# liyangSKD/slam-eslam

Measured on AMD Instinct MI355X. Metric: M particle-updates/s (predict+weight+resample) @ 1/2/4/8 MI355X, higher is better.
Workload: dtype f64; 1 GPU; configs[2]: 4194304 particles/GPU, 1 MI355X per rank, MLS 1000x1000 @0.1 m, 4 contacts, resample forced every step; particles_per_gpu=4194304, global_particles=4194304, parallelism=dp1 (particle shards)

## Files before the change

### include/eslam_detmath.h

```cpp
#ifndef ESLAM_DETMATH_H
#define ESLAM_DETMATH_H

#include <stdint.h>

#if defined(__HIPCC__)
#define DM_FN __host__ __device__ static inline __attribute__((always_inline))
#define DM_CONST static constexpr
#define DM_UNROLL _Pragma("unroll")
#else
#define DM_FN static inline
#define DM_CONST static const
#define DM_UNROLL
#endif

DM_FN uint64_t dm_bits(double x) { uint64_t u; __builtin_memcpy(&u, &x, 8); return u; }
DM_FN double dm_from_bits(uint64_t u) { double x; __builtin_memcpy(&x, &u, 8); return x; }
DM_FN uint32_t dm_fbits(float x) { uint32_t u; __builtin_memcpy(&u, &x, 4); return u; }
DM_FN int dm_isnan(double x) { return x != x; }
DM_FN int dm_isfinite(double x) { return (dm_bits(x) & 0x7ff0000000000000ull) != 0x7ff0000000000000ull; }
DM_FN double dm_fabs(double x) { return dm_from_bits(dm_bits(x) & 0x7fffffffffffffffull); }
DM_FN double dm_fma(double a, double b, double c) { return __builtin_fma(a, b, c); }
#if defined(__HIP_DEVICE_COMPILE__)
DM_FN double dm_fmak(double a, double b, double k)
{
// ... 1380 lines not shown
    uint64_t b = dm_bits(v);
    int e = (int)(b >> 52);
    if (e == 0x7ff) return 0x3fffffffffffffffull;
    if (e == 0) return 0;
    uint64_t m = (b & 0x000fffffffffffffull) | 0x0010000000000000ull;
    int sh = e - 1075 + shift;
    if (sh >= 10) return 0x3fffffffffffffffull;
    if (sh >= 0) return m << sh;
    if (sh <= -64) return 0;
    return m >> (-sh);
}

DM_FN uint64_t dm_fx61(double v) { return dm_fx_shift(v, 61); }

DM_FN uint64_t dm_count_draws_le(uint64_t c, uint64_t N, uint32_t xs, int shift)
{
    const unsigned __int128 prod = (unsigned __int128)c * N;
    const uint64_t kstar = (uint64_t)(prod >> shift);
    const uint64_t k0 = kstar >= 1 ? kstar - 1 : 0;
    if (k0 >= N) return N;
    uint64_t cnt = k0;
    uint32_t x = dm_mulmod31(dm_minstd_pow(k0 + 1), xs);
    const double dN = (double)N;
    for (uint64_t k = k0; k <= kstar + 1 && k < N; ++k) {
        const double u = dm_minstd_uniform(x);
        const uint64_t T = dm_fx_shift(((double)k + u) / dN, shift);
        if (T <= c) cnt = k + 1;
        else break;
        x = dm_minstd_next(x);
    }
    return cnt;
}


DM_FN int dm_fx128_limbs(double v, int scale, uint32_t limb[4])
{
    limb[0] = limb[1] = limb[2] = limb[3] = 0;
    if (!(v > 0.0)) return 0;
    uint64_t b = dm_bits(v);
    int e = (int)(b >> 52);
    uint64_t m;
    int ex;
    if (e == 0) { m = b & 0x000fffffffffffffull; ex = -1074; }
    else { m = (b & 0x000fffffffffffffull) | 0x0010000000000000ull; ex = e - 1075; }
    int sh = ex + scale;
    unsigned __int128 x;
    if (sh >= 0) {
        if (sh > 74) { limb[0] = limb[1] = limb[2] = 0xffffffffu; limb[3] = 0x7fffffffu; return 1; }
        x = (unsigned __int128)m << sh;
    } else {
        if (sh <= -64) return 0;
        x = (unsigned __int128)(m >> (-sh));
    }
    limb[0] = (uint32_t)x;
    limb[1] = (uint32_t)(x >> 32);
    limb[2] = (uint32_t)(x >> 64);
    limb[3] = (uint32_t)(x >> 96);
    return 0;
}

DM_FN double dm_limbs_to_double(const uint64_t L[4], int scale)
{
    uint32_t d[6];
    uint64_t carry = 0;
    for (int j = 0; j < 4; ++j) {
        uint64_t lo = (L[j] & 0xffffffffull) + carry;
// ... 307 lines not shown
```

### include/eslam_gpu.h

```cpp
#ifndef ESLAM_GPU_H
#define ESLAM_GPU_H

#include <stddef.h>
#include <stdint.h>

#ifdef __cplusplus
extern "C" {
#endif

#define ESLAM_ABI_VERSION 8

#define ESLAM_MAX_CONTACTS 32

#define ESLAM_OK 0
#define ESLAM_ERR_INVALID_ARG -1
#define ESLAM_ERR_NO_ENVIRONMENT -2
#define ESLAM_ERR_ZERO_MEAS_VAR -3
#define ESLAM_ERR_HASH_SAMPLE -4
#define ESLAM_ERR_NO_MLS_GRID -5
#define ESLAM_ERR_HIP -6
#define ESLAM_ERR_NOT_INITIALISED -7
#define ESLAM_ERR_UNSUPPORTED -8
#define ESLAM_ERR_OUT_OF_MEMORY -9
#define ESLAM_ERR_COMM -10
// ... 193 lines not shown

int eslam_gpu_scan_from_laser(eslam_ctx* ctx, const eslam_laser_scan* scan, const eslam_scan_params* params,
                              eslam_scan_info* info);
int eslam_gpu_scan_from_depth(eslam_ctx* ctx, const eslam_depth_image* image, const eslam_scan_params* params,
                              eslam_scan_info* info);
int eslam_gpu_scan_patches(eslam_ctx* ctx, eslam_scan_patch* out, uint64_t capacity, uint64_t* count);

typedef struct eslam_cpoint {
    double point[3];
    double zdiff, zvar;
    double prob;
} eslam_cpoint;

typedef struct eslam_particle_record {
    double position[2];
    double orientation, zpos, zsigma, mprob, weight;
    double meas_pos[3];
    double meas_theta;
    uint64_t index;
    uint32_t n_cpoints;
    uint8_t floating;
    uint8_t pad[3];
} eslam_particle_record;

int eslam_gpu_download_records(eslam_ctx* ctx, uint64_t first, uint64_t stride, uint64_t count,
                               eslam_particle_record* out, eslam_cpoint* cpoints, uint32_t max_cpoints);
int eslam_gpu_particle_count(const eslam_ctx* ctx, uint64_t* n);

int eslam_gpu_step(eslam_ctx* ctx, const eslam_step_input* in, int* updated);
int eslam_gpu_project(eslam_ctx* ctx, const eslam_step_input* in);
int eslam_gpu_update(eslam_ctx* ctx, const eslam_step_input* in);
int eslam_gpu_sync(eslam_ctx* ctx, eslam_update_info* info);
int eslam_gpu_debug_set_spin_limit(eslam_ctx* ctx, uint32_t polls);

int eslam_gpu_get_weights_sum(eslam_ctx* ctx, double* sum);
int eslam_gpu_normalize_weights(eslam_ctx* ctx, double* effective);
int eslam_gpu_resample(eslam_ctx* ctx);
typedef struct {
    uint64_t n_before;
    uint64_t n_after;
    uint64_t overruns;
    uint64_t dropped;
} eslam_resample_info;
int eslam_gpu_resample_stratified(eslam_ctx* ctx, uint64_t samples, eslam_resample_info* info);
int eslam_gpu_resample_multinomial(eslam_ctx* ctx, uint64_t samples, eslam_resample_info* info);
int eslam_gpu_get_best_particle_index(eslam_ctx* ctx, uint64_t* index);
int eslam_gpu_get_centroid(eslam_ctx* ctx, double position[3], double orientation[4]);

typedef struct eslam_rng_state {
    uint32_t minstd_x;
    uint32_t pad;
    uint64_t project_count;
    uint64_t init_count;
    uint64_t hash_count;
    double max_weight;
    double ud_pose[12];
    uint32_t libc_rand[34];
    uint32_t libc_rand_pos;
    uint32_t pad2;
} eslam_rng_state;
int eslam_gpu_get_rng_state(eslam_ctx* ctx, eslam_rng_state* st);
int eslam_gpu_set_rng_state(eslam_ctx* ctx, const eslam_rng_state* st);

#define ESLAM_SNAPSHOT_VERSION 1
#define ESLAM_SNAPSHOT_GRID 0x1u
#define ESLAM_SNAPSHOT_HASH 0x2u
// ... 71 lines not shown
```

### slam-eslam_amd/csrc/eslam_ctx.hip

```cpp
#include <hip/hip_runtime.h>
#include <rccl/rccl.h>
#include <dlfcn.h>

#include <math.h>
#include <stdlib.h>
#include <stdio.h>
#include <string.h>

#include <string>
#include <chrono>
#include <algorithm>
#include <atomic>
#include <functional>
#include <vector>

#include "eslam_internal.h"
#include "eslam_launch.h"
#include "eslam_buf.h"

using namespace eslam_dev;
using namespace eslam_buf;

namespace {

// ... 175 lines not shown

struct eslam_ctx {
    eslam_config cfg;
    int device = 0;
    hipStream_t stream = nullptr;
    bool own_stream = false;
    uint64_t n = 0, cap = 0;
    uint64_t gbase = 0, n_global = 0;
    DevState st[2] = {};
    ParticleBufs pt;
    uint64_t* fin_word = nullptr;
    uint32_t pub_stride = 0;
    uint64_t fin_epoch = 0;
    uint32_t scan_tag = 0;
    bool has_anc = false;
    LocalMaps lm = {};
    LocalMapBufs lmb;
    bool lm_ready = false;
    Pinned<ScanPatch> scan_host[2];
    Dev<ScanPatch> scan_dev[2];
    Event scan_ev[2];
    uint32_t scan_slot = 0;
    DebugRec dbg = {};
    DebugBufs dbgb;
    uint64_t dbg_cap = 0;
    bool dbg_valid = false;
    Dev<Shard> shards;
    Dev<Ctl> ctl;
    Pinned<Ctl> ctl_host;
    Pinned<uint32_t> fault_host;
    bool poisoned = false;
    bool poison_pages = false;
    uint32_t spin_limit = kSpinLimit;
    Dev<uint32_t> jump;
    uint32_t jump_n = 1;
    uint64_t jump_n_for = 0;
    Dev<double> scratch;
    Pinned<double> scratch_host;
    bool has_map = false;
    MapView map = {};
    GridBufs grid;
    uint64_t map_np = 0;
    uint64_t map_np_cap = 0;
    Dev<void> sm_mem;
    Dev<void> sm_x;
    Dev<void> pg_mem;
    GridBufs pg_out;
    uint64_t pg_out_cap = 0, pg_out_cells = 0;
    Dev<void> scan_mem;
    Dev<eslam_scan_patch> scan_out;
    uint64_t scan_count = 0;
    Pinned<void> snap_host[2];
    Dev<void> snap_dev[2];
    uint64_t snap_cap = 0;
    Event snap_ev[2];
    uint32_t maxp = 4;
    uint64_t proj_event = 0, init_event = 0, hash_event = 0;
    double ud_pose[12];
    double zcomp[4] = {1, 0, 0, 0};
    bool sharded = false;
    bool statics_sharded = false;
    eslam_comm comm = {};
    std::vector<uint64_t> gall;
    Dev<Shard> recs;
    Dev<uint64_t> mg;
    void* rccl = nullptr;
// ... 2069 lines not shown
    const double motion = sqrt(p.mu[0] * p.mu[0] + p.mu[1] * p.mu[1]) +
                          6.0 * sqrt(in->sample_cov[0] + in->sample_cov[4]);
    p.win_margin = reach + motion + 0.05;
    p.use_window = (c.flags & ESLAM_FLAG_NO_MAP_LDS) ? 0u : 1u;
    p.me2 = c.measurement_error * c.measurement_error;
    p.radius = c.contact_point_radius;
    p.corr = c.contact_likelihood_correction;
    p.min_contacts = c.min_contacts;
    p.use_shape = c.use_shape_update ? 1u : 0u;
    p.use_slip = c.use_slip_update ? 1u : 0u;
    p.n = ctx->n;
    p.gbase = ctx->gbase;
    p.n_global = ctx->n_global;
    p.J = dm_chunk_rows_cfg(ctx->n_global, ctx->cfg.sum_chunk_rows);
}

static uint32_t scan_items(uint64_t n)
{
    if (n <= (1ull << 18)) return 1u;
    return n <= (1ull << 19) ? 2u : (n <= (2ull << 20) ? 4u : (uint32_t)kScanItems);
}

static ScanParams scan_params(eslam_ctx* ctx, uint32_t phase_b, uint32_t normalize, bool multi)
{
    ScanParams sp;
    memset(&sp, 0, sizeof(sp));
    sp.spin_limit = ctx->spin_limit;
    sp.fault = ctx->fault_host;
    sp.n = ctx->n;
    sp.gbase = ctx->gbase;
    sp.n_global = ctx->n_global;
    sp.phase_b = phase_b;
    sp.normalize = normalize;
    sp.items = multi ? (uint32_t)kScanItems : scan_items(ctx->n);
    const uint64_t tile = (uint64_t)kBlock * sp.items;
    sp.ntiles = (uint32_t)((ctx->n + tile - 1) / tile);
    sp.pub_stride = ctx->pub_stride;
    return sp;
}

static FinParams fin_params(eslam_ctx* ctx, uint32_t mode)
{
    FinParams fp;
    memset(&fp, 0, sizeof(fp));
    fp.n_global = ctx->n_global;
    fp.min_effective = ctx->cfg.min_effective;
    fp.discount = ctx->cfg.discount_factor;
    fp.spread_threshold = ctx->cfg.spread_threshold;
    fp.mode = mode;
    if (ctx->jump_n_for != ctx->n_global) {
        ctx->jump_n = dm_minstd_pow(ctx->n_global);
        ctx->jump_n_for = ctx->n_global;
    }
    fp.minstd_jump_n = ctx->jump_n;
    return fp;
}

static int abort_pending_gather(eslam_ctx* ctx, hipError_t e, int rc = ESLAM_ERR_HIP)
{
    if (e != hipSuccess) fail(ctx, ESLAM_ERR_HIP, (std::string("sharded resample: ") + hipGetErrorString(e)).c_str());
    (void)hipMemsetAsync(ctx->pt.marks, 0, ctx->cap * 4, ctx->stream);
    (void)hipMemsetAsync(&ctx->ctl->flip, 0, sizeof(uint32_t), ctx->stream);
    (void)hipMemsetAsync(&ctx->ctl->gather, 0, sizeof(uint32_t), ctx->stream);
    (void)hipStreamSynchronize(ctx->stream);
    return rc;
}

// ... 439 lines not shown
    return launch_step(ctx, in, true, false);
}

extern "C" int eslam_gpu_update(eslam_ctx* ctx, const eslam_step_input* in)
{
    if (!ctx || !in) return ESLAM_ERR_INVALID_ARG;
    return launch_step(ctx, in, false, true);
}

extern "C" int eslam_gpu_step(eslam_ctx* ctx, const eslam_step_input* in, int* updated)
{
    if (!ctx || !in) return ESLAM_ERR_INVALID_ARG;
    const bool gate = update_gate(ctx->cfg.measurement_threshold_distance, ctx->cfg.measurement_threshold_angle, ctx->ud_pose,
                                  in->body2odometry_rot, in->body2odometry_trans) ||
                      in->ltc_count > 0;
    const int rc = launch_step(ctx, in, true, gate);
    if (rc) return rc;
    if (gate) {
        double R[9];
        q_to_mat(in->body2odometry_rot, R);
        for (int r = 0; r < 3; ++r) {
            for (int c = 0; c < 3; ++c) ctx->ud_pose[r * 4 + c] = R[r * 3 + c];
            ctx->ud_pose[r * 4 + 3] = in->body2odometry_trans[r];
        }
    }
    if (updated) *updated = gate ? 1 : 0;
    return ESLAM_OK;
}

extern "C" int eslam_gpu_debug_set_spin_limit(eslam_ctx* ctx, uint32_t polls)
{
    if (!ctx) return ESLAM_ERR_INVALID_ARG;
    ctx->spin_limit = polls;
    return ESLAM_OK;
}

extern "C" int eslam_gpu_sync(eslam_ctx* ctx, eslam_update_info* info)
{
    if (!ctx) return ESLAM_ERR_INVALID_ARG;
    if (const int rc_ = settle(ctx)) return rc_;
    int rc = read_ctl(ctx);
    if (rc) return rc;
    const Ctl& c = *ctx->ctl_host;
    if (info) {
        info->effective = c.eff;
        info->weight_sum = c.S;
        info->floating_weight = c.fw;
        info->max_weight = c.max_weight;
        info->data_particles = c.data_particles;
        info->total_points = c.total_points;
        info->resampled = (int32_t)c.resample;
        info->uniform_reset = (int32_t)c.uniform;
        info->resample_overruns = c.overruns;
        info->update_count = c.update_count;
        info->map_patches_dropped = c.map_dropped;
        info->map_stores_copied = c.map_copied;
        info->map_patches_covered = c.map_covered;
        info->map_stores_changed = c.map_changed;
        info->map_cells_written = c.map_written;
        info->map_pages_taken = c.map_taken;
        info->map_tiles_evicted = c.map_evicted;
        info->map_pages_free = c.pg_nfree > c.pg_cursor ? c.pg_nfree - c.pg_cursor : 0;
    }
    double acc[5];
    eslam_kernel_times& t = ctx->times;
    if (const uint32_t steps = ctx->timing ? ctx->ring.sums(acc) : 0) {
// ... 1426 lines not shown
```

### slam-eslam_amd/csrc/eslam_kernels.hip

```cpp
#include <hip/hip_runtime.h>
#include <type_traits>
#include <string.h>

#include "eslam_internal.h"
#include "eslam_launch.h"

namespace eslam_dev {

template <int O> __device__ __forceinline__ uint32_t xor_lane_u32(uint32_t v)
{
    static_assert(O == 1 || O == 2 || O == 4 || O == 8 || O == 16 || O == 32, "xor distance");
    if constexpr (O == 32) {
        const auto r = __builtin_amdgcn_permlane32_swap(v, v, false, false);
        return (threadIdx.x & 32u) ? r[0] : r[1];
    } else if constexpr (O == 16) {
        const auto r = __builtin_amdgcn_permlane16_swap(v, v, false, false);
        return (threadIdx.x & 16u) ? r[0] : r[1];
    } else if constexpr (O == 8) {
        const int t = __builtin_amdgcn_update_dpp(0, (int)v, 0x108, 0xf, 0x3, false);
        return (uint32_t)__builtin_amdgcn_update_dpp(t, (int)v, 0x118, 0xf, 0xc, false);
    } else if constexpr (O == 4) {
        const int t = __builtin_amdgcn_update_dpp(0, (int)v, 0x104, 0xf, 0x5, false);
        return (uint32_t)__builtin_amdgcn_update_dpp(t, (int)v, 0x114, 0xf, 0xa, false);
    } else if constexpr (O == 2) {
// ... 76 lines not shown
{
    return wave_butterfly(v, [](uint64_t a, uint64_t b) { return a + b; });
}

__device__ __forceinline__ uint64_t atomic_load_agent(const uint64_t* p)
{
    return __hip_atomic_load(p, __ATOMIC_RELAXED, __HIP_MEMORY_SCOPE_AGENT);
}

__device__ __forceinline__ void atomic_store_agent(uint64_t* p, uint64_t v)
{
    __hip_atomic_store(p, v, __ATOMIC_RELAXED, __HIP_MEMORY_SCOPE_AGENT);
}

#ifdef ESLAM_STAMPS
constexpr uint32_t kStampBlocks = 32768, kStampSlots = 8;
__device__ uint64_t g_stamps_k1[kStampBlocks][kStampSlots];
__device__ uint64_t g_stamps_k3[kStampBlocks][kStampSlots];
__device__ uint64_t g_stamps_mg[kStampBlocks][kStampSlots];
__device__ __forceinline__ uint64_t stamp_now()
{
    uint64_t t;
    asm volatile("s_memrealtime %0\n\ts_waitcnt lgkmcnt(0)" : "=s"(t)::"memory");
    return t;
}
__device__ uint32_t g_stamps_grid[3];
#define ESLAM_STAMP(arr, k) \
    do { \
        if (threadIdx.x == 0 && blockIdx.x < kStampBlocks) arr[blockIdx.x][(k)] = stamp_now(); \
        if ((k) == 0 && threadIdx.x == 0 && blockIdx.x == 0) g_stamps_grid[&arr == &g_stamps_k1 ? 0 : &arr == &g_stamps_k3 ? 1 : 2] = gridDim.x; \
    } while (0)
#else
#define ESLAM_STAMP(arr, k) do { } while (0)
#endif

typedef uint32_t su2 __attribute__((ext_vector_type(2)));
typedef uint32_t su4 __attribute__((ext_vector_type(4)));
typedef uint32_t su8 __attribute__((ext_vector_type(8)));
typedef uint32_t su16 __attribute__((ext_vector_type(16)));

#define KOFF(f) ((uint32_t)offsetof(K1Args, f))

__device__ __forceinline__ uint64_t kseg() { return (uint64_t)(uintptr_t)__builtin_amdgcn_kernarg_segment_ptr(); }

__device__ __forceinline__ su2 kl2(uint32_t off)
{
    su2 r;
    asm volatile("s_load_dwordx2 %0, %1, %2\n\ts_waitcnt lgkmcnt(0)" : "=&s"(r) : "s"(kseg()), "s"(off));
    return r;
}
__device__ __forceinline__ su4 kl4(uint32_t off)
{
    su4 r;
    asm volatile("s_load_dwordx4 %0, %1, %2\n\ts_waitcnt lgkmcnt(0)" : "=&s"(r) : "s"(kseg()), "s"(off));
    return r;
}
__device__ __forceinline__ su8 kl8(uint32_t off)
{
    su8 r;
    asm volatile("s_load_dwordx8 %0, %1, %2\n\ts_waitcnt lgkmcnt(0)" : "=&s"(r) : "s"(kseg()), "s"(off));
    return r;
}
__device__ __forceinline__ su16 kl16(uint32_t off)
{
    su16 r;
    asm volatile("s_load_dwordx16 %0, %1, %2\n\ts_waitcnt lgkmcnt(0)" : "=&s"(r) : "s"(kseg()), "s"(off));
// ... 2826 lines not shown

__device__ __forceinline__ void mark_segment(uint32_t* __restrict__ marks, uint32_t* __restrict__ tile_first,
                                             uint64_t lo, uint64_t hi, uint32_t v)
{
    marks[lo] = v;
    for (uint64_t t = (lo + kRow - 1) / kRow; t * kRow < hi; ++t) tile_first[t] = v - 1u;
}

constexpr int kSkew = 32;

__device__ __forceinline__ int skew(int k) { return k + k / kSkew; }

template <int ITEMS>
__device__ __forceinline__ uint64_t blocked_fx(const double* s_v, int shift, uint64_t (&c)[ITEMS])
{
    uint64_t run = 0;
#pragma unroll
    for (int r = 0; r < ITEMS; ++r) {
        run += fx_shift(s_v[skew((int)threadIdx.x * ITEMS + r)], shift);
        c[r] = run;
    }
    return run;
}

constexpr int kWaveChunks = 2;

template <int ITEMS> constexpr int wave_draws() { return 64 * ITEMS + 64 > 576 ? 64 * ITEMS + 64 : 576; }

__device__ __forceinline__ uint32_t draw_slot(uint32_t x) { return x + (x >> 3); }

template <int ITEMS> union K3Lds {
    double v[kBlock * ITEMS + kBlock * ITEMS / kSkew];
    uint64_t T[kWaves][wave_draws<ITEMS>() + wave_draws<ITEMS>() / 8];
};

template <int ITEMS>
__device__ __forceinline__ void flush_marks(uint32_t* __restrict__ marks, uint32_t* __restrict__ tile_first,
                                            const uint64_t (&seg_lo)[ITEMS], const uint64_t (&seg_hi)[ITEMS],
                                            const uint32_t (&val)[ITEMS])
{
#pragma unroll
    for (int q = 0; q < ITEMS; ++q) {
        const uint64_t lo = seg_lo[q], hi = seg_hi[q];
        if (hi <= lo) continue;
        marks[lo] = val[q];
        for (uint64_t t = (lo + kRow - 1) / kRow; t * kRow < hi; ++t) tile_first[t] = val[q] - 1u;
    }
}

__device__ __forceinline__ void flush_mark(uint32_t* __restrict__ marks, uint32_t* __restrict__ tile_first, uint64_t lo,
                                           uint64_t hi, uint32_t val)
{
    if (hi <= lo) return;
    marks[lo] = val;
    for (uint64_t t = (lo + kRow - 1) / kRow; t * kRow < hi; ++t) tile_first[t] = val - 1u;
}

constexpr uint64_t kPubMask = (1ull << 61) - 1;

__device__ __forceinline__ void publish_tile(uint64_t* pub, uint32_t stride, uint32_t tile, uint64_t w)
{
    if (threadIdx.x < kPubReplicas) atomic_store_agent(pub + (uint64_t)threadIdx.x * stride + tile, w);
}
__device__ __forceinline__ void publish_tile_1(uint64_t* pub, uint32_t stride, uint32_t tile, uint64_t w)
{
#pragma unroll
// ... 150 lines not shown
    const uint64_t kstar = kstar_of(c, N, shift);
    const uint64_t k0 = kstar >= 1 ? kstar - 1 : 0;
    if (k0 >= N) return 1u << 18;
    const uint64_t room = N - k0;
    uint32_t nd = kstar >= 1 ? 3u : 2u;
    nd = room < (uint64_t)nd ? (uint32_t)room : nd;
    return (uint32_t)(k0 - dlo) | (nd << 16);
}

__device__ __forceinline__ uint32_t draws_le_chunk(uint32_t w, uint64_t c, const uint64_t* sT, uint32_t rq0, uint32_t rq1)
{
    const uint32_t r0 = w & 0xffffu;
    const uint32_t nd = (w >> 16) & 3u;
#pragma unroll
    for (int d = 0; d < 3; ++d) {
        const uint32_t r = r0 + (uint32_t)d;
        const bool in = ((uint32_t)d < nd) & (r >= rq0) & (r < rq1);
        const uint64_t t = sT[draw_slot(in ? r - rq0 : 0u)];
        w |= (in && t <= c) ? 1u << (19 + d) : 0u;
    }
    return w;
}

__device__ __forceinline__ uint64_t count_from_window(uint32_t w, uint64_t dlo, uint64_t N)
{
    if ((w >> 18) & 1u) return N;
    const uint64_t k0 = dlo + (w & 0xffffu);
    const uint32_t le = (w >> 19) & 7u;
    const uint32_t lead = (le & 1u) ? ((le & 2u) ? ((le & 4u) ? 3u : 2u) : 1u) : 0u;
    return k0 + lead;
}

template <int ITEMS>
__device__ __forceinline__ void wave_counts(uint64_t base, uint64_t run, const uint64_t (&c)[ITEMS], uint64_t N, int shift,
                                            uint32_t xs, const uint32_t* __restrict__ jt, uint64_t* sT,
                                            uint64_t (&hi_r)[ITEMS], uint64_t& lo)
{
    const uint32_t lane = threadIdx.x & 63u;
    const double dN = (double)N, inv_N = 1.0 / dN;
    auto rfl64 = [](uint64_t v) {
        const uint32_t hi = (uint32_t)__builtin_amdgcn_readfirstlane((int)(uint32_t)(v >> 32));
        const uint32_t lo_ = (uint32_t)__builtin_amdgcn_readfirstlane((int)(uint32_t)v);
        return ((uint64_t)hi << 32) | (uint64_t)lo_;
    };
    const uint64_t wlo = rfl64(__shfl(base, 0, 64)), whi = rfl64(__shfl(base + run, 63, 64));
    const uint64_t ks_lo = kstar_of(wlo, N, shift), ks_hi = kstar_of(whi, N, shift);
    const uint64_t dlo = ks_lo >= 1 ? ks_lo - 1 : 0;
    const uint64_t dhi = ks_hi + 2 < N ? ks_hi + 2 : N;
    if (dlo >= dhi || dhi - dlo <= (uint64_t)kWaveChunks * wave_draws<ITEMS>()) {
        uint32_t win[ITEMS + 1];
#pragma unroll
        for (int r = 0; r <= ITEMS; ++r) win[r] = window_of(r < ITEMS ? base + c[r] : wlo, N, shift, dlo);
        const uint32_t a64 = jt[64], a_lane = jt[lane];
        for (uint64_t q0 = dlo; q0 < dhi; q0 += wave_draws<ITEMS>()) {
            const uint64_t q1 = dhi - q0 < (uint64_t)wave_draws<ITEMS>() ? dhi : q0 + wave_draws<ITEMS>();
            if (q0 + lane < q1) {
                uint32_t x = dm_mulmod31(dm_mulmod31(jump_pow(jt, q0 + 1), xs), a_lane);
#pragma unroll 4
                for (uint64_t k = q0 + lane; k < q1; k += 64) {
                    sT[draw_slot((uint32_t)(k - q0))] = draw_fx(k, x, dN, inv_N, shift);
                    x = dm_mulmod31(x, a64);
                }
            }
            __builtin_amdgcn_fence(__ATOMIC_RELEASE, "wavefront");
            __builtin_amdgcn_wave_barrier();
            __builtin_amdgcn_fence(__ATOMIC_ACQUIRE, "wavefront");
#pragma unroll
            for (int r = 0; r <= ITEMS; ++r)
                win[r] = draws_le_chunk(win[r], r < ITEMS ? base + c[r] : wlo, sT, (uint32_t)(q0 - dlo),
                                        (uint32_t)(q1 - dlo));
            __builtin_amdgcn_fence(__ATOMIC_RELEASE, "wavefront");
            __builtin_amdgcn_wave_barrier();
            __builtin_amdgcn_fence(__ATOMIC_ACQUIRE, "wavefront");
        }
#pragma unroll
        for (int r = 0; r < ITEMS; ++r) hi_r[r] = count_from_window(win[r], dlo, N);
        const uint64_t K0 = count_from_window(win[ITEMS], dlo, N);
        const uint64_t prev = __shfl_up(hi_r[ITEMS - 1], 1, 64);
        lo = lane == 0 ? K0 : prev;
    } else {
#pragma unroll
        for (int r = 0; r < ITEMS; ++r) hi_r[r] = count_draws_le(base + c[r], N, xs, shift, jt);
        const uint64_t K0 = count_draws_le(wlo, N, xs, shift, jt);
        const uint64_t prev = __shfl_up(hi_r[ITEMS - 1], 1, 64);
        lo = lane == 0 ? K0 : prev;
    }
}


template <int ITEMS, bool FUSED>
__global__ void __launch_bounds__(kBlock) __attribute__((amdgpu_waves_per_eu(ITEMS == 8 ? 6 : 1))) k_normalize_segments(DevState s0, DevState s1, ScanParams sp, Ctl* __restrict__ ctl,
                                                               uint64_t* __restrict__ tile_pub, uint32_t* __restrict__ marks,
                                                               uint32_t* __restrict__ tile_first,
                                                               const uint32_t* __restrict__ jt, FusedFin ff)
{
    __shared__ uint64_t s_wtot[kWaves], s_red[kWaves];
    __shared__ K3Lds<ITEMS> s_u;
    __shared__ uint64_t s_img[FUSED ? kCtlWords : 1];
    __shared__ uint32_t s_flag;
    const uint32_t tid = threadIdx.x, lane = tid & 63u, wave = tid >> 6;
    const uint32_t tile = blockIdx.x;
    ESLAM_STAMP(g_stamps_k3, 0);
    const uint64_t tagw = (uint64_t)sp.tag << 61;
    if (ctl->err & kFaultTimeout) {
        if (tid == 0) {
            if (FUSED && tile == 0) __hip_atomic_store(ff.fin_word, ff.epoch, __ATOMIC_RELEASE, __HIP_MEMORY_SCOPE_AGENT);
        }
        publish_tile(tile_pub, sp.pub_stride, tile, tagw);
        return;
    }
    if constexpr (FUSED) {
        if (tile == 0) {
            __shared__ FinLds s_fin;
            finalize_block(ff.shards, ff.nrec, ctl, ff.fp, s_fin);
            __syncthreads();
            if (tid == 0) {
                ctl->fin_epoch = ff.epoch;
                __hip_atomic_store(ff.fin_word, ff.epoch, __ATOMIC_RELEASE, __HIP_MEMORY_SCOPE_AGENT);
            }
        }
    }
// ... 38 lines not shown
    }
    __syncthreads();
    ESLAM_STAMP(g_stamps_k3, 3);
    const int shift = (int)sgpr_u32((uint32_t)cv->scan_shift);
    uint64_t c[ITEMS];
    const uint64_t run = blocked_fx(s_u.v, shift, c);
    uint64_t tincl = run;
#pragma unroll
    for (int o = 1; o < 64; o <<= 1) {
        const uint64_t t = __shfl_up(tincl, o, 64);
        if ((int)lane >= o) tincl += t;
    }
    if (lane == 63) s_wtot[wave] = tincl;
    __syncthreads();
    uint64_t wexcl = 0, agg = 0;
#pragma unroll
    for (int wv = 0; wv < kWaves; ++wv) {
        const uint64_t t = s_wtot[wv];
        if ((uint32_t)wv < wave) wexcl += t;
        agg += t;
    }
    ESLAM_STAMP(g_stamps_k3, 4);
    publish_tile(tile_pub, sp.pub_stride, tile, tagw | (agg & kPubMask));
    const uint64_t tb = tiles_before_pub(tile_pub + (uint64_t)(tile % kPubReplicas) * sp.pub_stride, tile, sp, s_red, ctl);
    if (tb == ~0ull) return;
    ESLAM_STAMP(g_stamps_k3, 5);
    const uint64_t base = tb + wexcl + (tincl - run);

    const uint64_t N = sp.n_global;
    const uint32_t xs = sgpr_u32(cv->minstd_start);
    const uint64_t i0 = t0 + (uint64_t)tid * ITEMS;
    uint64_t hi_r[ITEMS];
    uint64_t lo;
    wave_counts<ITEMS>(base, run, c, N, shift, xs, jt, s_u.T[wave], hi_r, lo);
    ESLAM_STAMP(g_stamps_k3, 6);
    if (i0 == 0) lo = 0;
#pragma unroll
    for (int r = 0; r < ITEMS; ++r) {
        const uint64_t i = i0 + r;
        if (i < sp.n) {
            uint64_t hi = hi_r[r];
            if (i == N - 1) {
                if (hi < N) atomicAdd((unsigned long long*)&ctl->overruns, (unsigned long long)(N - hi));
                hi = N;
            }
            flush_mark(marks, tile_first, lo, hi, (uint32_t)(i + 1));
            lo = hi;
        }
    }
    ESLAM_STAMP(g_stamps_k3, 7);
}

__device__ __forceinline__ void plan_bounds(const PlanParams& pp, const Ctl* ctl, const uint64_t* totals,
                                            const uint32_t* jt, uint64_t& off, uint64_t& O0, uint64_t& O1)
{
    off = 0;
    for (int r = 0; r < pp.rank; ++r) off += totals[r];
    const uint64_t N = pp.n_global;
    const uint32_t xs = ctl->minstd_start;
    const int shift = ctl->scan_shift;
    O0 = pp.rank == 0 ? 0 : count_draws_le(off, N, xs, shift, jt);
    O1 = pp.rank == pp.nranks - 1 ? N : count_draws_le(off + totals[pp.rank], N, xs, shift, jt);
}

__global__ void __launch_bounds__(kBlock) k_segments_multi(DevState s0, DevState s1, ScanParams sp, PlanParams pp,
                                                           Ctl* __restrict__ ctl, const uint64_t* __restrict__ tile_sum,
                                                           uint32_t* __restrict__ marks, uint32_t* __restrict__ tile_first,
// ... 11 lines not shown
        uint64_t c_lo = 0, c_hi = (pp.n_local + 64ull * pp.J - 1) / (64ull * pp.J);
        if (ctl->resample) {
            uint64_t off, O0, O1;
            plan_bounds(pp, ctl, totals, jt, off, O0, O1);
            own_chunks(O0, O1, pp.gbase[pp.rank], pp.n_local, pp.J, &c_lo, &c_hi);
        }
        pp.chunk_sel[0] = c_lo;
        pp.chunk_sel[1] = c_hi;
    }
    if (!ctl->resample) return;
    const uint32_t tid = threadIdx.x;
    const uint32_t tile = blockIdx.x;
    const DevState st = ctl->base ? s1 : s0;
    const uint64_t t0 = (uint64_t)tile * kScanTile;
#pragma unroll
    for (int r = 0; r < kScanItems; ++r) {
        const int k = r * kBlock + (int)tid;
        const uint64_t i = t0 + (uint64_t)k;
        s_v[skew(k)] = i < sp.n ? st.w[i] : 0.0;
    }
    __syncthreads();
    const int shift = ctl->scan_shift;
    uint64_t c[kScanItems];
    const uint64_t run = blocked_fx<kScanItems>(s_v, shift, c);
    const uint64_t tbase = tiles_before(tile_sum, tile, s_wtot) + block_excl(run, s_wtot);
    uint64_t off, O0, O1;
    plan_bounds(pp, ctl, totals, jt, off, O0, O1);
    const uint64_t base = off + tbase;
    const uint64_t N = pp.n_global;
    const uint64_t W0 = pp.gbase[pp.rank], W1 = pp.gbase[pp.rank + 1];
    const uint64_t i0 = t0 + (uint64_t)tid * kScanItems;
    uint64_t hi_r[kScanItems];
    uint64_t lo;
    wave_counts<kScanItems>(base, run, c, N, shift, ctl->minstd_start, jt, s_u.T[tid >> 6], hi_r, lo);
    if (i0 == 0) lo = O0;
    uint64_t seg_lo[kScanItems], seg_hi[kScanItems];
    uint32_t val[kScanItems];
#pragma unroll
    for (int r = 0; r < kScanItems; ++r) {
        const uint64_t i = i0 + r;
        seg_lo[r] = seg_hi[r] = 0;
        val[r] = kMarkOwn + 1u + (uint32_t)i;
        if (i >= sp.n) continue;
        uint64_t hi = hi_r[r];
        if (i + 1 == sp.n) {
            if (pp.rank == pp.nranks - 1 && hi < N)
                atomicAdd((unsigned long long*)&ctl->overruns, (unsigned long long)(N - hi));
            hi = O1;
        }
        const uint64_t a = lo > W0 ? lo : W0, b = hi < W1 ? hi : W1;
        if (a < b) { seg_lo[r] = a - W0; seg_hi[r] = b - W0; }
        if (lo < W0 || hi > W1) {
            range[i] = make_uint2((uint32_t)lo, (uint32_t)hi);
            if (hi > lo) {
                for (int d = 0; d < pp.nranks; ++d) {
                    if (d == pp.rank) continue;
                    const uint64_t Wd0 = pp.gbase[d], Wd1 = pp.gbase[d + 1];
                    const uint64_t Sd = O0 > Wd0 ? O0 : Wd0, Ed = O1 < Wd1 ? O1 : Wd1;
                    if (Sd >= Ed) continue;
                    if (lo <= Sd && Sd < hi) first_last[2 * d] = i;
                    if (lo <= Ed - 1 && Ed - 1 < hi) first_last[2 * d + 1] = i;
                }
            }
        }
        lo = hi;
    }
    flush_marks(marks, tile_first, seg_lo, seg_hi, val);
// ... 874 lines not shown
}

extern "C" int eslam_debug_k1_occupancy(int* blocks_per_cu, int lds)
{
    return hipOccupancyMaxActiveBlocksPerMultiprocessor(blocks_per_cu, k_project_weight<true, true, 4, true>, kBlock,
                                                        lds < 0 ? kStatsLds + kWindowLds : lds) == hipSuccess ? 0 : -1;
}

#ifdef ESLAM_STAMPS
extern "C" int eslam_gpu_debug_stamps_clear(void)
{
    void *a = nullptr, *b = nullptr, *c = nullptr, *g = nullptr;
    if (hipGetSymbolAddress(&a, HIP_SYMBOL(g_stamps_k1)) != hipSuccess || hipGetSymbolAddress(&b, HIP_SYMBOL(g_stamps_k3)) != hipSuccess ||
        hipGetSymbolAddress(&c, HIP_SYMBOL(g_stamps_mg)) != hipSuccess || hipGetSymbolAddress(&g, HIP_SYMBOL(g_stamps_grid)) != hipSuccess)
        return -1;
    const size_t bytes = sizeof(uint64_t) * kStampBlocks * kStampSlots;
    if (hipMemset(a, 0, bytes) != hipSuccess || hipMemset(b, 0, bytes) != hipSuccess || hipMemset(c, 0, bytes) != hipSuccess ||
        hipMemset(g, 0, 12) != hipSuccess)
        return -1;
    return hipDeviceSynchronize() == hipSuccess ? 0 : -1;
}

extern "C" int64_t eslam_gpu_debug_stamps(int which, uint64_t* out, uint64_t blocks)
{
    if (blocks > kStampBlocks) blocks = kStampBlocks;
    uint32_t grid[3] = {0, 0, 0};
    const hipError_t e = which == 1 ? hipMemcpyFromSymbol(out, HIP_SYMBOL(g_stamps_k1), blocks * kStampSlots * 8)
                         : which == 3 ? hipMemcpyFromSymbol(out, HIP_SYMBOL(g_stamps_k3), blocks * kStampSlots * 8)
                                      : hipMemcpyFromSymbol(out, HIP_SYMBOL(g_stamps_mg), blocks * kStampSlots * 8);
    if (e != hipSuccess || hipMemcpyFromSymbol(grid, HIP_SYMBOL(g_stamps_grid), sizeof(grid)) != hipSuccess) return -1;
    return (int64_t)grid[which == 1 ? 0 : which == 3 ? 1 : 2];
}
#endif
```

### slam-eslam_amd/eslam_amd.py

```python
import ctypes as C
import os

import numpy as np

import eslam_abi as A

HERE = os.path.dirname(os.path.abspath(__file__))
LIB_PATH = os.environ.get("ESLAM_GPU_LIB", os.path.join(HERE, "lib", "libeslam_gpu.so"))

_lib = None


class EslamError(RuntimeError):
    def __init__(self, code, msg):
        super().__init__(msg)
        self.code = code


def build_id():
    return load_library().eslam_gpu_build_id().decode()


def load_library(path=LIB_PATH):
    global _lib
# ... 32 lines not shown
        L.eslam_gpu_map_match.argtypes = [vp, C.POINTER(A.ScanPatch), C.c_uint32]
    if hasattr(L, "eslam_gpu_shared_map_update"):
        L.eslam_gpu_shared_map_update.argtypes = [vp, C.POINTER(A.ScanPatch), C.c_uint32, C.c_uint64,
                                                  C.POINTER(A.SharedMergeInfo)]
        L.eslam_gpu_map_size.argtypes = [vp, C.POINTER(C.c_uint32), C.POINTER(C.c_uint32), C.POINTER(C.c_uint64),
                                         C.POINTER(C.c_int)]
        L.eslam_gpu_get_map.argtypes = [vp, C.POINTER(C.c_uint32), C.POINTER(C.c_float), C.POINTER(C.c_float),
                                        C.POINTER(C.c_float), C.c_uint64]
    if hasattr(L, "eslam_gpu_shared_map_update_sharded"):
        L.eslam_gpu_shared_map_update_sharded.argtypes = [vp, C.POINTER(A.ScanPatch), C.c_uint32, C.c_uint64,
                                                          C.POINTER(A.SharedMergeInfo)]
    if hasattr(L, "eslam_gpu_scan_from_laser"):
        L.eslam_scan_params_default.argtypes = [C.POINTER(A.Config), C.POINTER(A.ScanParams)]
        L.eslam_gpu_scan_from_laser.argtypes = [vp, C.POINTER(A.LaserScan), C.POINTER(A.ScanParams), C.POINTER(A.ScanInfo)]
        L.eslam_gpu_scan_from_depth.argtypes = [vp, C.POINTER(A.DepthImage), C.POINTER(A.ScanParams), C.POINTER(A.ScanInfo)]
        L.eslam_gpu_scan_patches.argtypes = [vp, C.POINTER(A.ScanPatch), C.c_uint64, C.POINTER(C.c_uint64)]
    L.eslam_gpu_set_particle_maps.argtypes = [vp, C.c_int]
    L.eslam_gpu_get_particle_map.argtypes = [vp, C.c_uint64, C.POINTER(C.c_uint32), C.POINTER(C.c_float),
                                             C.POINTER(C.c_float), C.c_uint32, C.POINTER(C.c_uint32)]
    if hasattr(L, "eslam_gpu_get_particle_grid"):
        L.eslam_gpu_particle_grid_size.argtypes = [vp, C.c_uint64, C.POINTER(C.c_uint64)]
        L.eslam_gpu_get_particle_grid.argtypes = [vp, C.c_uint64, C.POINTER(C.c_uint32), C.POINTER(C.c_float),
                                                  C.POINTER(C.c_float), C.POINTER(C.c_float), C.c_uint64]
        L.eslam_gpu_adopt_particle_map.argtypes = [vp, C.c_uint64]
    L.eslam_gpu_download_records.argtypes = [vp, C.c_uint64, C.c_uint64, C.c_uint64, C.POINTER(A.ParticleRecord),
                                             C.POINTER(A.CPoint), C.c_uint32]
    L.eslam_gpu_particle_count.argtypes = [vp, C.POINTER(C.c_uint64)]
    L.eslam_gpu_step.argtypes = [vp, C.POINTER(A.StepInput), C.POINTER(C.c_int)]
    L.eslam_gpu_project.argtypes = [vp, C.POINTER(A.StepInput)]
    L.eslam_gpu_update.argtypes = [vp, C.POINTER(A.StepInput)]
    L.eslam_gpu_sync.argtypes = [vp, C.POINTER(A.UpdateInfo)]
    if hasattr(L, "eslam_gpu_debug_set_spin_limit"):
        L.eslam_gpu_debug_set_spin_limit.argtypes = [vp, C.c_uint32]
    L.eslam_gpu_get_weights_sum.argtypes = [vp, dp]
    L.eslam_gpu_normalize_weights.argtypes = [vp, dp]
    L.eslam_gpu_resample.argtypes = [vp]
    L.eslam_gpu_resample_stratified.argtypes = [vp, C.c_uint64, C.POINTER(A.ResampleInfo)]
    L.eslam_gpu_resample_multinomial.argtypes = [vp, C.c_uint64, C.POINTER(A.ResampleInfo)]
    L.eslam_gpu_get_best_particle_index.argtypes = [vp, C.POINTER(C.c_uint64)]
    L.eslam_gpu_get_centroid.argtypes = [vp, dp, dp]
    L.eslam_gpu_get_rng_state.argtypes = [vp, C.POINTER(A.RngState)]
    L.eslam_gpu_set_rng_state.argtypes = [vp, C.POINTER(A.RngState)]
    L.eslam_gpu_get_ancestors.argtypes = [vp, C.POINTER(C.c_uint32), C.c_uint64]
    L.eslam_gpu_enable_timing.argtypes = [vp, C.c_int]
    L.eslam_gpu_get_kernel_times.argtypes = [vp, C.POINTER(A.KernelTimes)]
    L.eslam_gpu_selftest_math.argtypes = [C.c_int, C.c_int, dp, dp, dp, C.c_uint64]
    up = C.POINTER(C.c_uint32)
    L.eslam_gpu_selftest_sort.argtypes = [C.c_int, up, up, C.c_uint64, up, up]
    if hasattr(L, "eslam_gpu_selftest_bm_radius"):
        L.eslam_gpu_selftest_bm_radius.argtypes = [C.c_int, C.POINTER(C.c_uint64)]
    L.eslam_gpu_set_comm.argtypes = [vp, C.POINTER(A.Comm), C.c_uint64, C.POINTER(C.c_uint64)]
    L.eslam_gpu_rccl_unique_id.argtypes = [C.POINTER(C.c_uint8)]
    L.eslam_gpu_set_comm_rccl.argtypes = [vp, C.c_int32, C.c_int32, C.POINTER(C.c_uint8), C.c_uint64,
                                          C.POINTER(C.c_uint64)]
    L.eslam_gpu_hash_create.argtypes = [vp]
    L.eslam_gpu_init_hash.argtypes = [vp, C.c_uint64]
    L.eslam_gpu_hash_info.argtypes = [vp, C.POINTER(C.c_uint64), C.POINTER(C.c_uint32)]
    L.eslam_gpu_hash_poses.argtypes = [vp, dp, dp, dp, dp, C.POINTER(C.c_int32)]
    for name, args in {**A.SNAPSHOT_PROTOTYPES, **A.SNAPSHOT_AT_PROTOTYPES}.items():
        if hasattr(L, name):
            getattr(L, name).argtypes = [vp] + args
    _lib = L
    return L


def _dv(v):
# ... 196 lines not shown
        n = C.c_uint64()
        bins = self.cfg.hash_slope_bins
        sizes = np.zeros(bins * bins, dtype=np.uint32)
        self._check(self.L.eslam_gpu_hash_info(self.h, C.byref(n), sizes.ctypes.data_as(C.POINTER(C.c_uint32))))
        return n.value, sizes

    def hash_poses(self):
        n, _ = self.hash_info()
        out = [np.zeros(n) for _ in range(4)]
        bucket = np.zeros(n, dtype=np.int32)
        ptr = lambda a: a.ctypes.data_as(C.POINTER(C.c_double))
        self._check(self.L.eslam_gpu_hash_poses(self.h, *[ptr(a) for a in out], bucket.ctypes.data_as(C.POINTER(C.c_int32))))
        return out + [bucket]

    def step(self, st):
        u = C.c_int(0)
        self._check(self.L.eslam_gpu_step(self.h, C.byref(st), C.byref(u)))
        return bool(u.value)

    def project(self, st):
        self._check(self.L.eslam_gpu_project(self.h, C.byref(st)))

    def update(self, st):
        self._check(self.L.eslam_gpu_update(self.h, C.byref(st)))

    def sync(self):
        info = A.UpdateInfo()
        self._check(self.L.eslam_gpu_sync(self.h, C.byref(info)))
        return info

    def debug_set_spin_limit(self, polls):
        self._check(self.L.eslam_gpu_debug_set_spin_limit(self.h, polls))

    def weights_sum(self):
        s = C.c_double()
        self._check(self.L.eslam_gpu_get_weights_sum(self.h, C.byref(s)))
        return s.value

    def normalize(self):
        e = C.c_double()
        self._check(self.L.eslam_gpu_normalize_weights(self.h, C.byref(e)))
        return e.value

    def resample(self):
        self._check(self.L.eslam_gpu_resample(self.h))

    def resample_stratified(self, samples):
        info = A.ResampleInfo()
        self._check(self.L.eslam_gpu_resample_stratified(self.h, samples, C.byref(info)))
        return info

    def resample_multinomial(self, samples):
        info = A.ResampleInfo()
        self._check(self.L.eslam_gpu_resample_multinomial(self.h, samples, C.byref(info)))
        return info

    def best_index(self):
        i = C.c_uint64()
        self._check(self.L.eslam_gpu_get_best_particle_index(self.h, C.byref(i)))
        return i.value

    def centroid(self):
        p = (C.c_double * 3)()
        q = (C.c_double * 4)()
        self._check(self.L.eslam_gpu_get_centroid(self.h, p, q))
        return list(p), list(q)
# ... 161 lines not shown
```

Baseline: 17760 M particle-updates/s.

## Add integer fast path for stratified resample draw counting with FP fallback

Adds an integer-only comparison that decides, for each cumulative-weight point, whether the k*-th stratified draw falls at or below it. The wave stages its MINSTD draws in LDS once, then each lane resolves its counts with fixed-point multiplies instead of the per-draw double-precision division loop. If any lane lands in an ambiguous margin, the whole wave falls back to the original floating-point routine, so results stay exact. This costs extra LDS space and a duplicated prologue, and it adds a debug hook for overriding scan items plus optional draw statistics.

```diff
diff --git a/include/eslam_detmath.h b/include/eslam_detmath.h
--- a/include/eslam_detmath.h
+++ b/include/eslam_detmath.h
@@ -1436,6 +1436,48 @@
     return cnt;
 }
 
+#define DM_DRAW_GT 0
+#define DM_DRAW_LE 1
+#define DM_DRAW_AMBIGUOUS (-1)
+#define DM_DRAW_SHIFT_MIN 54
+#define DM_DRAW_SHIFT_MAX 61
+
+DM_FN int dm_draw_shift_ok(int shift) { return shift >= DM_DRAW_SHIFT_MIN && shift <= DM_DRAW_SHIFT_MAX; }
+DM_FN uint64_t dm_draw_margin(int shift) { return 1ull << (shift - 51); }
+
+DM_FN void dm_draw_split(uint64_t c, uint64_t N, int shift, uint64_t* kstar, uint64_t* rem)
+{
+    const uint64_t lo = (uint64_t)(uint32_t)c * (uint32_t)N, hi = (c >> 32) * (uint64_t)(uint32_t)N;
+    const uint64_t top = hi + (lo >> 32);
+    const int s = (shift - 32) & 31;
+    *kstar = top >> s;
+    *rem = ((top & ((1ull << s) - 1ull)) << 32) | (uint64_t)(uint32_t)lo;
+}
+
+DM_FN uint64_t dm_mul_minstd_range_hi(uint64_t L)
+{
+    const uint64_t t = (uint64_t)(uint32_t)L * 2147483646u;
+    return (L >> 32) * 2147483646ull + (t >> 32);
+}
+
+DM_FN int dm_draw_decide(uint64_t kstar, uint64_t rem, uint64_t N, uint32_t x, int shift)
+{
+    const uint64_t mN = N << ((shift - 51) & 31);
+    const int edge = (kstar >= N) | (rem < mN) | ((1ull << (shift & 63)) - rem <= mN);
+    const uint64_t a = (uint64_t)(x - 1u) << ((shift - 32) & 31);
+    const int le = a <= dm_mul_minstd_range_hi(rem - mN);
+    const int gt = a > dm_mul_minstd_range_hi(rem + mN);
+    return (edge | !(le | gt)) ? DM_DRAW_AMBIGUOUS : le;
+}
+
+DM_FN int dm_draw_compare(uint64_t c, uint64_t N, uint32_t x, int shift)
+{
+    if (!dm_draw_shift_ok(shift) || (c >> 62) != 0 || N == 0 || (N >> 32) != 0) return DM_DRAW_AMBIGUOUS;
+    uint64_t kstar, rem;
+    dm_draw_split(c, N, shift, &kstar, &rem);
+    return dm_draw_decide(kstar, rem, N, x, shift);
+}
+
 
 DM_FN int dm_fx128_limbs(double v, int scale, uint32_t limb[4])
 {
diff --git a/include/eslam_gpu.h b/include/eslam_gpu.h
--- a/include/eslam_gpu.h
+++ b/include/eslam_gpu.h
@@ -249,6 +249,7 @@
 int eslam_gpu_update(eslam_ctx* ctx, const eslam_step_input* in);
 int eslam_gpu_sync(eslam_ctx* ctx, eslam_update_info* info);
 int eslam_gpu_debug_set_spin_limit(eslam_ctx* ctx, uint32_t polls);
+int eslam_gpu_debug_set_scan_items(eslam_ctx* ctx, uint32_t items);
 
 int eslam_gpu_get_weights_sum(eslam_ctx* ctx, double* sum);
 int eslam_gpu_normalize_weights(eslam_ctx* ctx, double* effective);
diff --git a/slam-eslam_amd/csrc/eslam_ctx.hip b/slam-eslam_amd/csrc/eslam_ctx.hip
--- a/slam-eslam_amd/csrc/eslam_ctx.hip
+++ b/slam-eslam_amd/csrc/eslam_ctx.hip
@@ -231,6 +231,7 @@
     bool poisoned = false;
     bool poison_pages = false;
     uint32_t spin_limit = kSpinLimit;
+    uint32_t debug_scan_items = 0;
     Dev<uint32_t> jump;
     uint32_t jump_n = 1;
     uint64_t jump_n_for = 0;
@@ -2366,7 +2367,7 @@
     sp.n_global = ctx->n_global;
     sp.phase_b = phase_b;
     sp.normalize = normalize;
-    sp.items = multi ? (uint32_t)kScanItems : scan_items(ctx->n);
+    sp.items = multi ? (uint32_t)kScanItems : (ctx->debug_scan_items ? ctx->debug_scan_items : scan_items(ctx->n));
     const uint64_t tile = (uint64_t)kBlock * sp.items;
     sp.ntiles = (uint32_t)((ctx->n + tile - 1) / tile);
     sp.pub_stride = ctx->pub_stride;
@@ -2872,6 +2873,14 @@
 {
     if (!ctx) return ESLAM_ERR_INVALID_ARG;
     ctx->spin_limit = polls;
+    return ESLAM_OK;
+}
+
+extern "C" int eslam_gpu_debug_set_scan_items(eslam_ctx* ctx, uint32_t items)
+{
+    if (!ctx) return ESLAM_ERR_INVALID_ARG;
+    if (items != 0 && items != 1 && items != 2 && items != 4 && items != (uint32_t)kScanItems) return ESLAM_ERR_INVALID_ARG;
+    ctx->debug_scan_items = items;
     return ESLAM_OK;
 }
 
diff --git a/slam-eslam_amd/csrc/eslam_kernels.hip b/slam-eslam_amd/csrc/eslam_kernels.hip
--- a/slam-eslam_amd/csrc/eslam_kernels.hip
+++ b/slam-eslam_amd/csrc/eslam_kernels.hip
@@ -132,6 +132,12 @@
     } while (0)
 #else
 #define ESLAM_STAMP(arr, k) do { } while (0)
+#endif
+#ifdef ESLAM_DRAW_STATS
+__device__ uint32_t g_draw_waves[2];
+#define ESLAM_DRAW_WAVE(k) do { if ((threadIdx.x & 63u) == 0) atomicAdd(&g_draw_waves[(k)], 1u); } while (0)
+#else
+#define ESLAM_DRAW_WAVE(k) do { } while (0)
 #endif
 
 typedef uint32_t su2 __attribute__((ext_vector_type(2)));
@@ -3024,6 +3030,7 @@
 template <int ITEMS> union K3Lds {
     double v[kBlock * ITEMS + kBlock * ITEMS / kSkew];
     uint64_t T[kWaves][wave_draws<ITEMS>() + wave_draws<ITEMS>() / 8];
+    uint32_t X[kWaves][2 * (wave_draws<ITEMS>() + wave_draws<ITEMS>() / 8)];
 };
 
 template <int ITEMS>
@@ -3240,9 +3247,9 @@
 }
 
 template <int ITEMS>
-__device__ __forceinline__ void wave_counts(uint64_t base, uint64_t run, const uint64_t (&c)[ITEMS], uint64_t N, int shift,
-                                            uint32_t xs, const uint32_t* __restrict__ jt, uint64_t* sT,
-                                            uint64_t (&hi_r)[ITEMS], uint64_t& lo)
+__device__ __forceinline__ void wave_counts_fp(uint64_t base, uint64_t run, const uint64_t (&c)[ITEMS], uint64_t N, int shift,
+                                               uint32_t xs, const uint32_t* __restrict__ jt, uint64_t* sT,
+                                               uint64_t (&hi_r)[ITEMS], uint64_t& lo)
 {
     const uint32_t lane = threadIdx.x & 63u;
     const double dN = (double)N, inv_N = 1.0 / dN;
@@ -3295,6 +3302,66 @@
     }
 }
 
+template <int ITEMS>
+__device__ __forceinline__ void wave_counts(uint64_t base, uint64_t run, const uint64_t (&c)[ITEMS], uint64_t N, int shift,
+                                            uint32_t xs, const uint32_t* __restrict__ jt, uint64_t* sT, uint32_t* sX,
+                                            uint64_t (&hi_r)[ITEMS], uint64_t& lo)
+{
+    ESLAM_DRAW_WAVE(0);
+    if (dm_draw_shift_ok(shift)) {
+        const uint32_t lane = threadIdx.x & 63u;
+        auto rfl64 = [](uint64_t v) {
+            const uint32_t hi = (uint32_t)__builtin_amdgcn_readfirstlane((int)(uint32_t)(v >> 32));
+            const uint32_t lo_ = (uint32_t)__builtin_amdgcn_readfirstlane((int)(uint32_t)v);
+            return ((uint64_t)hi << 32) | (uint64_t)lo_;
+        };
+        const uint64_t wlo = rfl64(__shfl(base, 0, 64)), whi = rfl64(__shfl(base + run, 63, 64));
+        const uint64_t ks_lo = kstar_of(wlo, N, shift), ks_hi = kstar_of(whi, N, shift);
+        const uint64_t dlo = ks_lo >= 1 ? ks_lo - 1 : 0;
+        const uint64_t dhi = ks_hi + 2 < N ? ks_hi + 2 : N;
+        if (dlo < dhi && dhi - dlo <= (uint64_t)wave_draws<ITEMS>()) {
+            if (dlo + lane < dhi) {
+                const uint32_t a64 = jt[64];
+                uint32_t x = dm_mulmod31(dm_mulmod31(jump_pow(jt, dlo + 1), xs), jt[lane]);
+#pragma unroll 4
+                for (uint64_t k = dlo + lane; k < dhi; k += 64) {
+                    sX[draw_slot((uint32_t)(k - dlo))] = x;
+                    x = dm_mulmod31(x, a64);
+                }
+            }
+            __builtin_amdgcn_fence(__ATOMIC_RELEASE, "wavefront");
+            __builtin_amdgcn_wave_barrier();
+            __builtin_amdgcn_fence(__ATOMIC_ACQUIRE, "wavefront");
+            bool amb = false;
+            uint32_t cnt[ITEMS + 1];
+            const uint32_t span = (uint32_t)(dhi - dlo);
+#pragma unroll
+            for (int r = 0; r <= ITEMS; ++r) {
+                uint64_t ks, rem;
+                dm_draw_split(r < ITEMS ? base + c[r] : wlo, N, shift, &ks, &rem);
+                const uint32_t rel = (uint32_t)ks - (uint32_t)dlo;
+                const bool staged = rel < span;
+                const uint32_t x = sX[draw_slot(staged ? rel : 0u)];
+                const int d = dm_draw_decide(ks, rem, N, x, shift);
+                amb |= !staged | (d < 0);
+                cnt[r] = (uint32_t)ks + (d > 0 ? 1u : 0u);
+            }
+            if (__builtin_amdgcn_ballot_w64(amb) == 0) {
+#pragma unroll
+                for (int r = 0; r < ITEMS; ++r) hi_r[r] = cnt[r];
+                const uint64_t prev = __shfl_up(hi_r[ITEMS - 1], 1, 64);
+                lo = lane == 0 ? cnt[ITEMS] : prev;
+                return;
+            }
+            __builtin_amdgcn_fence(__ATOMIC_RELEASE, "wavefront");
+            __builtin_amdgcn_wave_barrier();
+            __builtin_amdgcn_fence(__ATOMIC_ACQUIRE, "wavefront");
+        }
+    }
+    ESLAM_DRAW_WAVE(1);
+    wave_counts_fp<ITEMS>(base, run, c, N, shift, xs, jt, sT, hi_r, lo);
+}
+
 
 template <int ITEMS, bool FUSED>
 __global__ void __launch_bounds__(kBlock) __attribute__((amdgpu_waves_per_eu(ITEMS == 8 ? 6 : 1))) k_normalize_segments(DevState s0, DevState s1, ScanParams sp, Ctl* __restrict__ ctl,
@@ -3399,7 +3466,7 @@
     const uint64_t i0 = t0 + (uint64_t)tid * ITEMS;
     uint64_t hi_r[ITEMS];
     uint64_t lo;
-    wave_counts<ITEMS>(base, run, c, N, shift, xs, jt, s_u.T[wave], hi_r, lo);
+    wave_counts<ITEMS>(base, run, c, N, shift, xs, jt, s_u.T[wave], s_u.X[wave], hi_r, lo);
     ESLAM_STAMP(g_stamps_k3, 6);
     if (i0 == 0) lo = 0;
 #pragma unroll
@@ -3477,7 +3544,7 @@
     const uint64_t i0 = t0 + (uint64_t)tid * kScanItems;
     uint64_t hi_r[kScanItems];
     uint64_t lo;
-    wave_counts<kScanItems>(base, run, c, N, shift, ctl->minstd_start, jt, s_u.T[tid >> 6], hi_r, lo);
+    wave_counts<kScanItems>(base, run, c, N, shift, ctl->minstd_start, jt, s_u.T[tid >> 6], s_u.X[tid >> 6], hi_r, lo);
     if (i0 == 0) lo = O0;
     uint64_t seg_lo[kScanItems], seg_hi[kScanItems];
     uint32_t val[kScanItems];
@@ -4418,3 +4485,12 @@
     return (int64_t)grid[which == 1 ? 0 : which == 3 ? 1 : 2];
 }
 #endif
+
+#ifdef ESLAM_DRAW_STATS
+extern "C" int eslam_gpu_debug_draw_waves(uint32_t* out, int clear)
+{
+    const uint32_t zero[2] = {0, 0};
+    if (hipDeviceSynchronize() != hipSuccess || hipMemcpyFromSymbol(out, HIP_SYMBOL(g_draw_waves), 8) != hipSuccess) return -1;
+    return !clear || hipMemcpyToSymbol(HIP_SYMBOL(g_draw_waves), zero, 8) == hipSuccess ? 0 : -1;
+}
+#endif
diff --git a/slam-eslam_amd/eslam_amd.py b/slam-eslam_amd/eslam_amd.py
--- a/slam-eslam_amd/eslam_amd.py
+++ b/slam-eslam_amd/eslam_amd.py
@@ -88,6 +88,8 @@
     L.eslam_gpu_sync.argtypes = [vp, C.POINTER(A.UpdateInfo)]
     if hasattr(L, "eslam_gpu_debug_set_spin_limit"):
         L.eslam_gpu_debug_set_spin_limit.argtypes = [vp, C.c_uint32]
+    if hasattr(L, "eslam_gpu_debug_set_scan_items"):
+        L.eslam_gpu_debug_set_scan_items.argtypes = [vp, C.c_uint32]
     L.eslam_gpu_get_weights_sum.argtypes = [vp, dp]
     L.eslam_gpu_normalize_weights.argtypes = [vp, dp]
     L.eslam_gpu_resample.argtypes = [vp]
@@ -350,6 +352,9 @@
     def debug_set_spin_limit(self, polls):
         self._check(self.L.eslam_gpu_debug_set_spin_limit(self.h, polls))
 
+    def debug_set_scan_items(self, items):
+        self._check(self.L.eslam_gpu_debug_set_scan_items(self.h, items))
+
     def weights_sum(self):
         s = C.c_double()
         self._check(self.L.eslam_gpu_get_weights_sum(self.h, C.byref(s)))
```

Result: faster. 18300 M particle-updates/s (median of 6 runs) (+3.1%).
